# heng-hw/SpaCap3D

Hardware: AMD Instinct MI355X
Metric: scenes/sec (40k pts, 256 proposals) fwd+bwd (higher is better)
Workload: dtype f32; 1 GPU; cfg2: synthetic ScanRefer-shaped scans, 40000 pts x (xyz+1 ch), 256 proposals, 8 scenes/GPU; full training step (SpaCapNet fwd + loss + bwd + grad all-reduce + Adam); global_batch=8, parallelism=dp1, hip_graph=True, fps_prefetch_side_stream=True, prefetch_as_graph=True, reserved_cus_forward=8, geometry_prefetch=True, deferred_weight_gradients=True, params=9290918, allreduce_bytes=35572416

## Files before the change

include/spacap_hip.h:

```cpp
#ifndef SPACAP_HIP_H
#define SPACAP_HIP_H

#include <stddef.h>
#include <stdint.h>

#ifdef __cplusplus
extern "C" {
#endif

#define SPACAP_ABI_VERSION 5

#define SPACAP_OK 0
#define SPACAP_E_INVALID (-1)
#define SPACAP_E_LAUNCH (-2)
#define SPACAP_E_NO_DEVICE (-3)

typedef void *spacap_stream_t;

int spacap_abi_version(void);
const char *spacap_last_error(void);
int spacap_device_count(void);

int spacap_opt_n_threads(int work_size);

// ... 361 lines not shown
  float eps;
  uint64_t seed;
  const uint64_t *seed_dev;
  const float *res;
  float *x_out;
  const float *ln_a;
  const float *ln_b;
  float *n_out;
  float *stats;
  const float *x_ln;
  const float *g;
  float *part;
  const float *w2;
  const float *bias2;
  float *out2;
  int n2;
  int nparts;
  const float *attn_out;
  float *delta_out;
  int lq;
} spacap_tf_rows_args;
int spacap_tf_rows_f32(const spacap_tf_rows_args *args, spacap_stream_t stream);
int spacap_tf_rows_parts(long R);
int spacap_tf_ffn1_f32(const float *x, const float *W, const float *bias, long R, int N, float drop_p, uint64_t seed,
                       const uint64_t *seed_dev, float *h, spacap_stream_t stream);
int spacap_tf_ffn_f32(int mode, const float *x, const float *Wa, const float *Wb, const float *bias, const float *y, long R, int dff,
                      float drop_p, uint64_t seed, const uint64_t *seed_dev, float *hid, float *part, spacap_stream_t stream);
long spacap_tf_ffn_pieces_elems(int dff);
int spacap_tf_ffn_split_f32(const float *const *w1, const float *const *w2, void *const *pieces, int nlayers, int dff,
                            spacap_stream_t stream);
int spacap_tf_ffn_bf3_f32(int mode, const float *x, const void *pieces, const float *bias, const float *y, long R, int dff, float drop_p,
                          uint64_t seed, const uint64_t *seed_dev, float *hid, float *part, spacap_stream_t stream);
int spacap_decode_attn_f32(const float *qkv, float *kcache, float *vcache, long R, int h, int d_k, int T, int t, float scale,
                           float *out, spacap_stream_t stream);
size_t spacap_decode_word_workspace_bytes(long R, int V);
int spacap_decode_word_f32(const float *x, const void *Wp, const float *bias, long R, int V, const float *lut, float scale,
                           const float *pe_row, int64_t *ys, int ys_ld, int t_out, float *x_next, void *workspace,
                           spacap_stream_t stream);
int spacap_tf_gemm_splits(long R, int K, int N);
int spacap_tf_gemm_f32(const float *a, const float *W, long R, int K, int N, int trans_w, int nsplit, float *out,
                       spacap_stream_t stream);
int spacap_tf_dgrad_mask_f32(const float *g, const float *W, const float *y, float scale, long R, int K, int N, float *out,
                             spacap_stream_t stream);

int spacap_conv1x1_cm_supported(int CI, int CO, long N);
int spacap_conv1x1_cm_f32(int mode, const float *W, const float *in, const float *bias, int B, int CI, int CO, long N,
// ... 66 lines not shown
```

spacap3d_amd/_native.py:

```python
import ctypes
import os

import torch

_HERE = os.path.dirname(os.path.abspath(__file__))
LIB_PATH = os.path.join(_HERE, "lib", "libspacap_hip.so")
ABI_VERSION = 5

_i = ctypes.c_int
_l = ctypes.c_long
_f = ctypes.c_float
_p = ctypes.c_void_p
_u64 = ctypes.c_uint64

SIGNATURES = {
    "spacap_abi_version": (_i, []),
    "spacap_last_error": (ctypes.c_char_p, []),
    "spacap_device_count": (_i, []),
    "spacap_opt_n_threads": (_i, [_i]),
    "spacap_fps_workspace_bytes": (ctypes.c_size_t, [_i, _i]),
    "spacap_fps_f32": (_i, [_p, _i, _i, _i, _p, _p, _p]),
    "spacap_gather_points_f32": (_i, [_p, _p, _i, _i, _i, _i, _p, _p]),
    "spacap_gather_points_grad_f32": (_i, [_p, _p, _i, _i, _i, _i, _p, _p]),
    "spacap_ball_query_f32": (_i, [_p, _p, _i, _i, _i, _f, _i, _p, _p]),
# ... 141 lines not shown
    "spacap_rel_tail_bwd_nparts": (_i, [_l]),
    "spacap_rel_tail_bwd_f32": (_i, [_p, _p, _p, _l, _p, _p, _p]),
    "spacap_conv1x1_wgrad_slabs": (_i, [_i, _i, _i, _i]),
    "spacap_conv1x1_wgrad_f32": (_i, [_p, _p, _i, _i, _i, _i, _p, _p]),
    "spacap_conv1x1_wgrad_slabs_batched": (_i, [_i, _i, _i, _i]),
    "spacap_conv1x1_wgrad_batched_f32": (_i, [_p, _p, _p, _p, _p, _p, _p, _p, _p, _i, _p]),
    "spacap_linear_rows_supported": (_i, [_l, _i, _i]),
    "spacap_linear_rows_f32": (_i, [_p, _p, _p, _l, _i, _i, _i, _p, _p]),
    "spacap_linear_wgrad_slabs": (_i, [_l, _i, _i]),
    "spacap_linear_wgrad_f32": (_i, [_p, _p, _l, _i, _i, _i, _p, _p]),
    "spacap_linear_wgrad_nslab_f32": (_i, [_p, _p, _l, _i, _i, _i, _i, _p, _p]),
    "spacap_linear_wgrad_slabs_batched": (_i, [_l, _i, _i]),
    "spacap_linear_wgrad_batched_f32": (_i, [_p, _p, _p, _p, _p, _p, _p, _p, _i, _p]),
    "spacap_layernorm_fwd_f32": (_i, [_p, _p, _p, _l, _i, _f, _p, _p, _p]),
    "spacap_layernorm_bwd_workspace_bytes": (ctypes.c_size_t, [_l, _i]),
    "spacap_layernorm_bwd_f32": (_i, [_p, _p, _p, _p, _l, _i, _f, _p, _p, _p, _p, _p]),
    "spacap_layernorm_bwd_add_f32": (_i, [_p, _p, _p, _p, _p, _l, _i, _f, _p, _p, _p, _p, _p]),
    "spacap_proposal_decode_fwd_f32": (_i, [_p, _p, _p, _p, _i, _i, _i, _i, _i, _p, _p, _p, _p, _p, _p, _p, _p, _p]),
    "spacap_proposal_decode_bwd_f32": (_i, [_p, _p, _p, _p, _p, _i, _i, _i, _i, _i, _p, _p]),
    "spacap_loss_tail_fwd_f32": (_i, [_p, _p, _p, _p, _p, _p, _i, _p, _p, _p]),
    "spacap_loss_tail_bwd_f32": (_i, [_p, _p, _p, _p, _p]),
    "spacap_tf_rows_f32": (_i, [_p, _p]),
    "spacap_tf_rows_parts": (_i, [_l]),
    "spacap_tf_ffn1_f32": (_i, [_p, _p, _p, _l, _i, _f, _u64, _p, _p, _p]),
    "spacap_tf_ffn_f32": (_i, [_i, _p, _p, _p, _p, _p, _l, _i, _f, _u64, _p, _p, _p, _p]),
    "spacap_tf_ffn_pieces_elems": (_l, [_i]),
    "spacap_tf_ffn_split_f32": (_i, [_p, _p, _p, _i, _i, _p]),
    "spacap_tf_ffn_bf3_f32": (_i, [_i, _p, _p, _p, _p, _l, _i, _f, _u64, _p, _p, _p, _p]),
    "spacap_decode_attn_f32": (_i, [_p, _p, _p, _l, _i, _i, _i, _i, _f, _p, _p]),
    "spacap_decode_word_workspace_bytes": (ctypes.c_size_t, [_l, _i]),
    "spacap_decode_word_f32": (_i, [_p, _p, _p, _l, _i, _p, _f, _p, _p, _i, _i, _p, _p, _p]),
    "spacap_tf_gemm_splits": (_i, [_l, _i, _i]),
    "spacap_tf_gemm_f32": (_i, [_p, _p, _l, _i, _i, _i, _i, _p, _p]),
    "spacap_tf_dgrad_mask_f32": (_i, [_p, _p, _p, _f, _l, _i, _i, _p, _p]),
    "spacap_mha_fwd_f32": (_i, [_p, _p, _p] + [_l] * 9 + [_p, _l, _l, _p, _l, _l, _l]
                           + [_i] * 5 + [_f, _f, _u64, _p, _p, _p, _p, _p]),
    "spacap_mha_bwd_workspace_bytes": (ctypes.c_size_t, [_i, _i, _i]),
    "spacap_mha_bwd_delta_f32": (_i, [_p, _p, _p] + [_l] * 9 + [_p, _l, _l, _p, _l, _l, _l]
                                 + [_i] * 5 + [_f, _f, _u64, _p, _p, _p, _p, _p, _p, _p, _l, _p]),
    "spacap_mha_bwd_f32": (_i, [_p, _p, _p] + [_l] * 9 + [_p, _l, _l, _p, _l, _l, _l]
                           + [_i] * 5 + [_f, _f, _u64, _p, _p, _p, _p, _p, _p, _p, _p, _l, _p]),
}


class TfRowsArgs(ctypes.Structure):
    _fields_ = [("mode", _i), ("R", _l), ("a1", _p), ("w1", _p), ("bias1", _p), ("k1", _i), ("drop_p", _f), ("eps", _f),
                ("seed", _u64), ("seed_dev", _p), ("res", _p), ("x_out", _p), ("ln_a", _p), ("ln_b", _p), ("n_out", _p),
                ("stats", _p), ("x_ln", _p), ("g", _p), ("part", _p), ("w2", _p), ("bias2", _p), ("out2", _p), ("n2", _i), ("nparts", _i), ("attn_out", _p), ("delta_out", _p), ("lq", _i)]


def _load():
    if not os.path.exists(LIB_PATH):
        raise ImportError(
            f"{LIB_PATH} not found: the HIP extension is not built. Run "
            "`python -c 'import __graft_entry__ as g; g.build()'` (or `make -C spacap3d_amd/csrc`). "
            "spacap3d_amd has no CPU or PyTorch fallback for its native operators.")
    lib = ctypes.CDLL(LIB_PATH)
    for name, (res, args) in SIGNATURES.items():
        fn = getattr(lib, name)
        fn.restype = res
        fn.argtypes = args
    got = lib.spacap_abi_version()
    if got != ABI_VERSION:
        raise ImportError(f"libspacap_hip.so ABI {got} != expected {ABI_VERSION}: rebuild the extension")
    return lib


lib = _load()


def check(rc: int, what: str) -> None:
# ... 196 lines not shown
```

spacap3d_amd/tf_layer.py:

```python
import ctypes

import torch
from torch.autograd import Function

from ._native import TfRowsArgs, check, grad_slot, lib, linear_wgrad_partials, sum_slabs

D_MODEL = 128
ENABLED = True


def supported(d_model, d_ff):
    return d_model == D_MODEL and d_ff >= 128 and d_ff % 128 == 0


def _p(t):
    return t.data_ptr() if t is not None else None


def _rows(mode, R, dev, **kw):
    a = TfRowsArgs()
    a.mode, a.R = mode, R
    a.k1 = int(kw.pop("k1", 0))
    a.n2 = int(kw.pop("n2", 0))
    a.nparts = int(kw.pop("nparts", 0))
    a.lq = int(kw.pop("lq", 0))
    a.drop_p = float(kw.pop("drop_p", 0.0))
    a.eps = float(kw.pop("eps", 1e-6))
    a.seed = int(kw.pop("seed", 0))
    a.seed_dev = None
    if a.drop_p > 0.0:
        from .attention import rng_state
# ... 231 lines not shown
            if g_hpre is not None and g_parts is not None:
                gh, gp = g_hpre.reshape(R, dff).contiguous(), g_parts.contiguous()
                _rows(1, R, dev, a1=gp, nparts=gp.shape[0], **kw)
                dW1, db1 = _linear_grads(gh, n2, W1)
            elif g_hpre is not None:
                gh = g_hpre.reshape(R, dff).contiguous()
                parts, S = _split_product(gh, W1, False)
                _rows(1, R, dev, a1=parts, nparts=S, **kw)
                dW1, db1 = _linear_grads(gh, n2, W1)
            else:
                _rows(1, R, dev, g=torch.zeros(R, D_MODEL, dtype=torch.float32, device=dev), **kw)
            dln_a, dln_b = _ln_param_grads(part)
            dWo, dbo = _linear_grads(dy1, a.reshape(R, D_MODEL), Wo)
            dqkv = torch.empty_like(qc)
            base, gb = qc.data_ptr(), dqkv.data_ptr()
            check(lib.spacap_mha_bwd_delta_f32(base, base + hd * es, base + 2 * hd * es, *strides, *strides, *strides, _p(mask_u8),
                                               mask_sb, mask_sq, None, 0, 0, 0, B, heads, L, L, dk, scale, p_att, seed_att,
                                               rng_state(dev).data_ptr() if p_att > 0.0 else None, lse.data_ptr(), da.data_ptr(),
                                               delta.data_ptr(), gb, gb + hd * es, gb + 2 * hd * es, three, st),
                  "spacap_mha_bwd_delta_f32")
        return (dqkv, dx1, None, None, None, None, None, None, dWo, dbo, dln_a, dln_b, dW1, db1, None, None, None, None, None, None)


class Ffn2Ln(Function):

    @staticmethod
    def forward(ctx, h, parts, x1, W1, W2, b2, ln_a, ln_b, eps, p_sub, p_ffn, seed3, pw, pb, *routing):
        if not h.is_cuda:
            raise RuntimeError("CPU not supported")
        hc, xr, pc = h.contiguous(), x1.contiguous(), parts.contiguous()
        R, dev = xr.numel() // D_MODEL, xr.device
        last = pw is None
        with torch.cuda.device(dev):
            x2, n, stats = _new(dev, *xr.shape), _new(dev, *xr.shape), _new(dev, R, 2)
            kw = dict(a1=pc, nparts=pc.shape[0], bias1=b2, drop_p=p_sub, seed=seed3, res=xr, x_out=x2, ln_a=ln_a, ln_b=ln_b,
                      eps=eps, n_out=n, stats=stats)
            qkv = None
            if not last:
                qkv = _new(dev, *xr.shape[:-1], pw.shape[0])
                kw.update(w2=pw, bias2=pb, n2=pw.shape[0], out2=qkv)
            _rows(0, R, dev, **kw)
        ctx.save_for_backward(hc, x2, n, stats, ln_a, W1, W2, pw)
        ctx.meta = (float(eps), float(p_sub), float(p_ffn), int(seed3), last, [int(r.shape[0]) for r in routing[:3]])
        ctx.set_materialize_grads(False)
        return (n,) if last else (x2, qkv)

# ... 41 lines not shown


def stack_supported(layers, x):
    if not (ENABLED and x.is_cuda and x.dtype == torch.float32 and x.shape[-1] == D_MODEL and len(layers) > 0):
        return False
    for l in layers:
        ff, sa = l.feed_forward, l.self_attn
        if getattr(l, "early_guide", True) is not True or sa.h * sa.d_k != D_MODEL:
            return False
        if not supported(ff.w_1.in_features, ff.w_1.out_features) or ff.w_2.bias is None or ff.w_1.bias is None:
            return False
        if any(li.bias is None or not li.weight.is_contiguous() for li in sa.linears):
            return False
    return True


def decode_supported(layers, x, n_words):
    if not stack_supported(layers, x) or n_words + 1 > 32:
        return False
    dff = layers[0].feed_forward.w_1.out_features
    return all(l.self_attn.h == 8 and l.self_attn.d_k == 16 and l.feed_forward.w_1.out_features == dff for l in layers)


def run_stack(layers, final_norm, x, mask):
    from .attention import _next_seed, _prep_mask, self_attention_packed

    def drop(m):
        return float(m.p) if m.training else 0.0

    def seed(p):
        return _next_seed() if p > 0.0 else 0

    sub = lambda l: (l.sublayer[0], l.sublayer[-1])
    l0 = layers[0]
    if x.numel() // x.shape[-1] > FFN_BF3_MIN_ROWS:
        refresh_ffn_pieces(layers)
    pw, pb, routing = _packed(l0.self_attn)
    qkv, xres = LnQkv.apply(x, l0.sublayer[0].norm.a_2, l0.sublayer[0].norm.b_2, l0.sublayer[0].norm.eps, pw, pb, *routing)
    out = None
    for i, l in enumerate(layers):
        sa, ff = l.self_attn, l.feed_forward
        s_att, s_ffn = sub(l)
        need_p = sa.keep_value if sa.store_attn is None else (sa.store_attn or sa.keep_value)
        p1, pf, p3 = drop(s_att.dropout), drop(ff.dropout), drop(s_ffn.dropout)
        wo = sa.linears[-1]
        tail = (wo.weight, wo.bias, s_ffn.norm.a_2, s_ffn.norm.b_2, ff.w_1.weight, ff.w_1.bias, ff.w_2.weight, s_ffn.norm.eps, p1, pf)
        if not need_p and sa.d_k == 16 and sa.h == 8:
            B_, L_ = qkv.shape[0], qkv.shape[1]
            m8, msb, msq = _prep_mask(mask, B_, L_, L_)
            pa = float(sa.dropout.p) if sa.dropout.training else 0.0
            sa.attn = None
            x1, h, parts = AttnFfn1.apply(qkv, xres, m8, msb, msq, sa.h, pa, seed(pa), *tail, seed(p1), seed(pf))
        else:
            a, sa.attn = self_attention_packed(qkv, sa.h, mask=mask, dropout_p=sa.dropout.p, training=sa.dropout.training,
                                               need_p=need_p)
            if sa.keep_value:
                hd = sa.h * sa.d_k
                sa.value = qkv[..., 2 * hd:].view(qkv.shape[0], -1, sa.h, sa.d_k).transpose(1, 2)
            x1, h, parts = AttnOutFfn1.apply(a, xres, *tail, seed(p1), seed(pf))
# ... 80 lines not shown
```

Before: 1151 scenes/s.

## Fuse short-sequence transformer layer into single per-scene block kernels

Adds a new HIP kernel pair that, for sequences up to 32 tokens, runs the FFN-residual sum, LayerNorm, QKV projection, attention, output projection, residual and second LayerNorm in one workgroup per scene, with a matching fused backward. The Python stack routes through it when shapes are supported. The aim is to cut the many small kernel launches and global-memory round trips of the short transformer stack. In exchange it adds a large specialised kernel with one block per batch element, which on a batch of 8 leaves most CUs idle and may run slower than the multi-kernel path.

```diff
diff --git a/include/spacap_hip.h b/include/spacap_hip.h
--- a/include/spacap_hip.h
+++ b/include/spacap_hip.h
@@ -407,6 +407,56 @@
 } spacap_tf_rows_args;
 int spacap_tf_rows_f32(const spacap_tf_rows_args *args, spacap_stream_t stream);
 int spacap_tf_rows_parts(long R);
+typedef struct {
+  int B, L;
+  const uint64_t *seed_dev;
+  const float *parts;
+  int nparts;
+  const float *bias0;
+  float drop0;
+  uint64_t seed0;
+  const float *x;
+  float *x0;
+  const float *ln1_a;
+  const float *ln1_b;
+  float eps1;
+  float *n1;
+  float *stats1;
+  const float *wqkv;
+  const float *bqkv;
+  float *qkv;
+  const uint8_t *mask;
+  long mask_sb, mask_sq;
+  float att_scale;
+  float drop_att;
+  uint64_t seed_att;
+  float *attn;
+  float *lse;
+  const float *wo;
+  const float *bo;
+  float drop1;
+  uint64_t seed1;
+  const float *ln2_a;
+  const float *ln2_b;
+  float eps2;
+  float *x1;
+  float *n2;
+  float *stats2;
+  const float *gparts;
+  int ngparts;
+  const float *g_x1;
+  float *dy1;
+  float *part2;
+  float *dqkv;
+  float *dx;
+  float *part1;
+  float *dy0;
+} spacap_tf_short_args;
+int spacap_tf_short_supported(int L, int d_model, int h, int d_k);
+int spacap_tf_short_parts(int B);
+long spacap_tf_short_lds_bytes(int backward);
+int spacap_tf_short_fwd_f32(const spacap_tf_short_args *args, spacap_stream_t stream);
+int spacap_tf_short_bwd_f32(const spacap_tf_short_args *args, spacap_stream_t stream);
 int spacap_tf_ffn1_f32(const float *x, const float *W, const float *bias, long R, int N, float drop_p, uint64_t seed,
                        const uint64_t *seed_dev, float *h, spacap_stream_t stream);
 int spacap_tf_ffn_f32(int mode, const float *x, const float *Wa, const float *Wb, const float *bias, const float *y, long R, int dff,
diff --git a/spacap3d_amd/_native.py b/spacap3d_amd/_native.py
--- a/spacap3d_amd/_native.py
+++ b/spacap3d_amd/_native.py
@@ -187,6 +187,11 @@
     "spacap_loss_tail_bwd_f32": (_i, [_p, _p, _p, _p, _p]),
     "spacap_tf_rows_f32": (_i, [_p, _p]),
     "spacap_tf_rows_parts": (_i, [_l]),
+    "spacap_tf_short_supported": (_i, [_i, _i, _i, _i]),
+    "spacap_tf_short_parts": (_i, [_i]),
+    "spacap_tf_short_lds_bytes": (_l, [_i]),
+    "spacap_tf_short_fwd_f32": (_i, [_p, _p]),
+    "spacap_tf_short_bwd_f32": (_i, [_p, _p]),
     "spacap_tf_ffn1_f32": (_i, [_p, _p, _p, _l, _i, _f, _u64, _p, _p, _p]),
     "spacap_tf_ffn_f32": (_i, [_i, _p, _p, _p, _p, _p, _l, _i, _f, _u64, _p, _p, _p, _p]),
     "spacap_tf_ffn_pieces_elems": (_l, [_i]),
@@ -212,6 +217,15 @@
     _fields_ = [("mode", _i), ("R", _l), ("a1", _p), ("w1", _p), ("bias1", _p), ("k1", _i), ("drop_p", _f), ("eps", _f),
                 ("seed", _u64), ("seed_dev", _p), ("res", _p), ("x_out", _p), ("ln_a", _p), ("ln_b", _p), ("n_out", _p),
                 ("stats", _p), ("x_ln", _p), ("g", _p), ("part", _p), ("w2", _p), ("bias2", _p), ("out2", _p), ("n2", _i), ("nparts", _i), ("attn_out", _p), ("delta_out", _p), ("lq", _i)]
+
+
+class TfShortArgs(ctypes.Structure):
+    _fields_ = [("B", _i), ("L", _i), ("seed_dev", _p), ("parts", _p), ("nparts", _i), ("bias0", _p), ("drop0", _f), ("seed0", _u64),
+                ("x", _p), ("x0", _p), ("ln1_a", _p), ("ln1_b", _p), ("eps1", _f), ("n1", _p), ("stats1", _p), ("wqkv", _p),
+                ("bqkv", _p), ("qkv", _p), ("mask", _p), ("mask_sb", _l), ("mask_sq", _l), ("att_scale", _f), ("drop_att", _f),
+                ("seed_att", _u64), ("attn", _p), ("lse", _p), ("wo", _p), ("bo", _p), ("drop1", _f), ("seed1", _u64), ("ln2_a", _p),
+                ("ln2_b", _p), ("eps2", _f), ("x1", _p), ("n2", _p), ("stats2", _p), ("gparts", _p), ("ngparts", _i), ("g_x1", _p),
+                ("dy1", _p), ("part2", _p), ("dqkv", _p), ("dx", _p), ("part1", _p), ("dy0", _p)]
 
 
 def _load():
diff --git a/spacap3d_amd/csrc/tf_short.hip b/spacap3d_amd/csrc/tf_short.hip
--- /dev/null
+++ b/spacap3d_amd/csrc/tf_short.hip
@@ -0,0 +1,704 @@
+#include <math.h>
+
+#include "common.hpp"
+#include "mfma.hpp"
+
+namespace {
+
+using namespace spacap::mfma;
+using f32x2 = float __attribute__((ext_vector_type(2)));
+
+constexpr int D = 128;
+constexpr int NH = 8, DK = 16;
+constexpr int LMAX = 32;
+constexpr int LDT = D + 8;
+constexpr int QS = 3 * D + 4;
+constexpr int NTHR = 512;
+
+constexpr size_t FWD_LDS = sizeof(float) * (LMAX * LDT + LMAX * QS + 2 * 8 * 16);
+constexpr size_t BWD_LDS = sizeof(float) * (2 * LMAX * LDT + LMAX * QS + 2 * 8 * 16 + NH * LMAX);
+
+__device__ __forceinline__ f32x2 ld2(const float *p) { return *reinterpret_cast<const f32x2 *>(p); }
+
+struct DropSeed {
+  unsigned lo, hi;
+};
+__device__ __forceinline__ DropSeed make_seed(unsigned long long seed, const unsigned long long *seed_dev) {
+  const unsigned long long s = seed + (seed_dev ? *seed_dev * 0x9E3779B97F4A7C15ull : 0ull);
+  return DropSeed{(unsigned)s, (unsigned)(s >> 32)};
+}
+__device__ __forceinline__ unsigned hash32(unsigned long long idx, DropSeed s) {
+  unsigned h = (unsigned)idx ^ s.lo;
+  h += ((unsigned)(idx >> 32) ^ s.hi) * 0x9E3779B1u;
+  h ^= h >> 16;
+  h *= 0x85EBCA6Bu;
+  h ^= h >> 13;
+  h *= 0xC2B2AE35u;
+  h ^= h >> 16;
+  return h;
+}
+
+struct Drop {
+  unsigned thresh;
+  float scale;
+  unsigned long long seed;
+};
+
+struct ShortArgs {
+  int B, L;
+  const unsigned long long *seed_dev;
+  const float *parts;
+  int nparts;
+  const float *bias0;
+  Drop d0;
+  const float *x;
+  float *x0;
+  const float *ln1_a, *ln1_b;
+  float eps1;
+  float *n1, *stats1;
+  const float *wqkv, *bqkv;
+  float *qkv;
+  const uint8_t *mask;
+  long mask_sb, mask_sq;
+  float att_scale;
+  Drop da;
+  float *attn, *lse;
+  const float *wo, *bo;
+  Drop d1;
+  const float *ln2_a, *ln2_b;
+  float eps2;
+  float *x1, *n2, *stats2;
+  const float *gparts;
+  int ngparts;
+  const float *g_x1;
+  float *dy1, *part2, *dqkv, *dx, *part1, *dy0;
+};
+
+struct Place {
+  int lane, w, w4, mt, l15, lg, rl;
+  bool valid;
+  long row, rowc;
+};
+__device__ __forceinline__ Place place(int b, int L) {
+  Place p;
+  p.lane = threadIdx.x & 63, p.w = threadIdx.x >> 6, p.w4 = p.w & 3, p.mt = p.w >> 2, p.l15 = p.lane & 15, p.lg = p.lane >> 4;
+  p.rl = 16 * p.mt + p.l15;
+  p.valid = p.rl < L;
+  p.row = (long)b * L + p.rl;
+  p.rowc = p.valid ? p.row : (long)b * L + L - 1;
+  return p;
+}
+
+__device__ __forceinline__ float red4(const float *s_red, int k, int mt, int l15) {
+  const float *r = s_red + (k * 8 + 4 * mt) * 16 + l15;
+  return (r[0] + r[16]) + (r[32] + r[48]);
+}
+
+__device__ __forceinline__ f32x4 sum_parts(const float *pp, size_t ps, int nparts) {
+  f32x4 a = ld4(pp);
+  int sidx = 1;
+  for (; sidx + 7 < nparts; sidx += 8) {
+    f32x4 t[8];
+#pragma unroll
+    for (int u = 0; u < 8; ++u) t[u] = ld4(pp + (sidx + u) * ps);
+#pragma unroll
+    for (int u = 0; u < 8; ++u) a += t[u];
+  }
+  for (; sidx + 3 < nparts; sidx += 4) {
+    const f32x4 t0 = ld4(pp + sidx * ps), t1 = ld4(pp + (sidx + 1) * ps), t2 = ld4(pp + (sidx + 2) * ps), t3 = ld4(pp + (sidx + 3) * ps);
+    a += t0, a += t1, a += t2, a += t3;
+  }
+  for (; sidx < nparts; ++sidx) a += ld4(pp + sidx * ps);
+  return a;
+}
+
+__device__ __forceinline__ void ln_fwd(const Place &pl, const int *cb, const float (&xo)[2][4], const float *ln_a, const float *ln_b,
+                                       float eps, float *n_out, float *stats, float *s_red, float (&t_out)[2][4]) {
+  float s = 0.f;
+#pragma unroll
+  for (int g = 0; g < 2; ++g)
+#pragma unroll
+    for (int t = 0; t < 4; ++t) s += xo[g][t];
+  s += __shfl_xor(s, 16);
+  s += __shfl_xor(s, 32);
+  if (pl.lg == 0) s_red[(0 * 8 + pl.w) * 16 + pl.l15] = s;
+  __syncthreads();
+  const float mu = red4(s_red, 0, pl.mt, pl.l15) / (float)D;
+  float q = 0.f;
+#pragma unroll
+  for (int g = 0; g < 2; ++g)
+#pragma unroll
+    for (int t = 0; t < 4; ++t) {
+      const float c = xo[g][t] - mu;
+      q += c * c;
+    }
+  q += __shfl_xor(q, 16);
+  q += __shfl_xor(q, 32);
+  if (pl.lg == 0) s_red[(1 * 8 + pl.w) * 16 + pl.l15] = q;
+  __syncthreads();
+  const float var = red4(s_red, 1, pl.mt, pl.l15) / (float)(D - 1);
+  const float r = 1.0f / (sqrtf(var) + eps);
+#pragma unroll
+  for (int g = 0; g < 2; ++g) {
+    const f32x4 a4 = ld4(ln_a + cb[g]), b4 = ld4(ln_b + cb[g]);
+#pragma unroll
+    for (int t = 0; t < 4; ++t) t_out[g][t] = a4[t] * ((xo[g][t] - mu) * r) + b4[t];
+    if (pl.valid) st4(n_out + (size_t)pl.row * D + cb[g], f32x4{t_out[g][0], t_out[g][1], t_out[g][2], t_out[g][3]});
+  }
+  if (pl.valid && pl.w4 == 0 && pl.lg == 0) {
+    stats[pl.row * 2] = mu;
+    stats[pl.row * 2 + 1] = r;
+  }
+}
+
+__device__ __forceinline__ float logit(const ShortArgs &P, float dot, int b, int q, int key, bool &masked) {
+  const int L = P.L;
+  float s = dot * P.att_scale;
+  const int qc = q < L ? q : L - 1, kc = key < L ? key : L - 1;
+  masked = false;
+  if (P.mask && P.mask[b * P.mask_sb + qc * P.mask_sq + kc] == 0) {
+    s = -1e9f;
+    masked = true;
+  }
+  if (key >= L) s = -INFINITY;
+  return s;
+}
+__device__ __forceinline__ bool keep_att(const ShortArgs &P, DropSeed sd, int b, int hh, int q, int key) {
+  if (P.da.thresh == 0u) return true;
+  const unsigned long long idx = (((unsigned long long)b * NH + hh) * P.L + q) * (unsigned long long)P.L + key;
+  return hash32(idx, sd) >= P.da.thresh;
+}
+
+__global__ __launch_bounds__(NTHR) void tf_short_fwd_kernel(const ShortArgs P) {
+  extern __shared__ __attribute__((aligned(16))) unsigned char smem_raw[];
+  float *s_t = reinterpret_cast<float *>(smem_raw);
+  float *s_qkv = s_t + LMAX * LDT;
+  float *s_red = s_qkv + LMAX * QS;
+  const int b = blockIdx.x, L = P.L;
+  const Place pl = place(b, L);
+  const int l15 = pl.l15, lg = pl.lg, w4 = pl.w4;
+  const long R = (long)P.B * L;
+  int cb[2];
+#pragma unroll
+  for (int g = 0; g < 2; ++g) cb[g] = 32 * w4 + 16 * g + 4 * lg;
+
+  float xo[2][4], t_out[2][4];
+  {
+    const DropSeed sd = make_seed(P.d0.seed, P.seed_dev);
+#pragma unroll
+    for (int g = 0; g < 2; ++g) {
+      const f32x4 r4 = ld4(P.x + (size_t)pl.rowc * D + cb[g]);
+      if (P.parts != nullptr) {
+        const f32x4 v = sum_parts(P.parts + (size_t)pl.rowc * D + cb[g], (size_t)R * D, P.nparts);
+        f32x4 b4 = {0.f, 0.f, 0.f, 0.f};
+        if (P.bias0) b4 = ld4(P.bias0 + cb[g]);
+#pragma unroll
+        for (int t = 0; t < 4; ++t) {
+          float a = v[t] + b4[t];
+          if (P.d0.thresh != 0u) {
+            const bool keep = hash32((unsigned long long)pl.row * D + cb[g] + t, sd) >= P.d0.thresh;
+            a = keep ? a * P.d0.scale : 0.f;
+          }
+          xo[g][t] = r4[t] + a;
+        }
+        if (pl.valid) st4(P.x0 + (size_t)pl.row * D + cb[g], f32x4{xo[g][0], xo[g][1], xo[g][2], xo[g][3]});
+      } else {
+#pragma unroll
+        for (int t = 0; t < 4; ++t) xo[g][t] = r4[t];
+      }
+    }
+  }
+  ln_fwd(pl, cb, xo, P.ln1_a, P.ln1_b, P.eps1, P.n1, P.stats1, s_red, t_out);
+
+#pragma unroll
+  for (int g = 0; g < 2; ++g) st4(&s_t[pl.rl * LDT + cb[g]], f32x4{t_out[g][0], t_out[g][1], t_out[g][2], t_out[g][3]});
+  __syncthreads();
+  {
+    f32x4 at[8];
+#pragma unroll
+    for (int q = 0; q < 8; ++q) at[q] = ld4(&s_t[pl.rl * LDT + 16 * q + 4 * lg]);
+    const int n00 = 96 * w4;
+    const float *wp = P.wqkv + (size_t)(n00 + l15) * D + 4 * lg;
+#pragma unroll
+    for (int jt = 0; jt < 96; jt += 32) {
+      f32x4 x[8], y[8];
+#pragma unroll
+      for (int q = 0; q < 8; ++q) x[q] = ld4(wp + (size_t)jt * D + 16 * q), y[q] = ld4(wp + (size_t)(jt + 16) * D + 16 * q);
+      f32x4 acc0 = {0.f, 0.f, 0.f, 0.f}, acc1 = {0.f, 0.f, 0.f, 0.f};
+#pragma unroll
+      for (int q = 0; q < 8; ++q)
+#pragma unroll
+        for (int i = 0; i < 4; ++i) {
+          acc0 = MFMA16(x[q][i], at[q][i], acc0);
+          acc1 = MFMA16(y[q][i], at[q][i], acc1);
+        }
+      const int c0 = n00 + jt + 4 * lg;
+      if (P.bqkv) acc0 += ld4(P.bqkv + c0), acc1 += ld4(P.bqkv + c0 + 16);
+      if (pl.valid) {
+        st4(P.qkv + (size_t)pl.row * 3 * D + c0, acc0);
+        st4(P.qkv + (size_t)pl.row * 3 * D + c0 + 16, acc1);
+      }
+      st4(&s_qkv[pl.rl * QS + c0], acc0);
+      st4(&s_qkv[pl.rl * QS + c0 + 16], acc1);
+    }
+  }
+  __syncthreads();
+
+  {
+    const DropSeed sd = make_seed(P.da.seed, P.seed_dev);
+    const int lq = l15;
+#pragma unroll
+    for (int tk = 0; tk < 2; ++tk) {
+      const int id = 2 * pl.w + tk, hh = id >> 1, q0 = (id & 1) * 16;
+      if (q0 >= L) continue;
+      const int q = q0 + lq, qc = q < L ? q : L - 1;
+      const float *qp = s_qkv + qc * QS + hh * DK;
+      float qreg[DK / 4];
+#pragma unroll
+      for (int s = 0; s < DK / 4; ++s) qreg[s] = qp[4 * s + lg];
+      f32x4 acc[2];
+#pragma unroll
+      for (int t = 0; t < 2; ++t) {
+        acc[t] = f32x4{0.f, 0.f, 0.f, 0.f};
+        if (16 * t < L) {
+          const int key = 16 * t + lq;
+          const float *kp = s_qkv + (key < L ? key : L - 1) * QS + D + hh * DK;
+#pragma unroll
+          for (int s = 0; s < DK / 4; ++s) acc[t] = MFMA16(kp[4 * s + lg], qreg[s], acc[t]);
+        }
+      }
+      float m = -INFINITY;
+#pragma unroll
+      for (int t = 0; t < 2; ++t)
+#pragma unroll
+        for (int r = 0; r < 4; ++r) {
+          bool masked;
+          acc[t][r] = logit(P, acc[t][r], b, q, 16 * t + 4 * lg + r, masked);
+          m = fmaxf(m, acc[t][r]);
+        }
+      m = fmaxf(m, __shfl_xor(m, 16));
+      m = fmaxf(m, __shfl_xor(m, 32));
+      float l = 0.f;
+#pragma unroll
+      for (int t = 0; t < 2; ++t)
+#pragma unroll
+        for (int r = 0; r < 4; ++r) {
+          acc[t][r] = expf(acc[t][r] - m);
+          l += acc[t][r];
+        }
+      l += __shfl_xor(l, 16);
+      l += __shfl_xor(l, 32);
+      if (lg == 0 && q < L) {
+        float *st = P.lse + (((size_t)b * NH + hh) * L + q) * 2;
+        st[0] = m;
+        st[1] = l;
+      }
+#pragma unroll
+      for (int t = 0; t < 2; ++t)
+#pragma unroll
+        for (int r = 0; r < 4; ++r) {
+          float pv = acc[t][r] / l;
+          if (!keep_att(P, sd, b, hh, q, 16 * t + 4 * lg + r)) pv = 0.f; else pv *= P.da.scale;
+          acc[t][r] = pv;
+        }
+      f32x4 o = {0.f, 0.f, 0.f, 0.f};
+#pragma unroll
+      for (int t = 0; t < 2; ++t) {
+        if (16 * t < L) {
+#pragma unroll
+          for (int r = 0; r < 4; ++r) {
+            const int key = 16 * t + 4 * lg + r;
+            const float *vp = s_qkv + (key < L ? key : L - 1) * QS + 2 * D + hh * DK;
+            o = MFMA16(acc[t][r], vp[lq], o);
+          }
+        }
+      }
+#pragma unroll
+      for (int rr = 0; rr < 4; ++rr) {
+        const int qo = q0 + 4 * lg + rr;
+        s_t[qo * LDT + hh * DK + lq] = o[rr];
+        if (qo < L) P.attn[((size_t)b * L + qo) * D + hh * DK + lq] = o[rr];
+      }
+    }
+  }
+  __syncthreads();
+
+  {
+    f32x4 at[8], x[8], y[8];
+    const float *wp0 = P.wo + (size_t)(32 * w4 + l15) * D + 4 * lg, *wp1 = wp0 + (size_t)16 * D;
+#pragma unroll
+    for (int q = 0; q < 8; ++q) x[q] = ld4(wp0 + 16 * q), y[q] = ld4(wp1 + 16 * q), at[q] = ld4(&s_t[pl.rl * LDT + 16 * q + 4 * lg]);
+    f32x4 acc[2] = {f32x4{0.f, 0.f, 0.f, 0.f}, f32x4{0.f, 0.f, 0.f, 0.f}};
+#pragma unroll
+    for (int q = 0; q < 8; ++q)
+#pragma unroll
+      for (int i = 0; i < 4; ++i) {
+        acc[0] = MFMA16(x[q][i], at[q][i], acc[0]);
+        acc[1] = MFMA16(y[q][i], at[q][i], acc[1]);
+      }
+    const DropSeed sd = make_seed(P.d1.seed, P.seed_dev);
+#pragma unroll
+    for (int g = 0; g < 2; ++g) {
+      f32x4 b4 = {0.f, 0.f, 0.f, 0.f};
+      if (P.bo) b4 = ld4(P.bo + cb[g]);
+#pragma unroll
+      for (int t = 0; t < 4; ++t) {
+        float a = acc[g][t] + b4[t];
+        if (P.d1.thresh != 0u) {
+          const bool keep = hash32((unsigned long long)pl.row * D + cb[g] + t, sd) >= P.d1.thresh;
+          a = keep ? a * P.d1.scale : 0.f;
+        }
+        xo[g][t] = xo[g][t] + a;
+      }
+      if (pl.valid) st4(P.x1 + (size_t)pl.row * D + cb[g], f32x4{xo[g][0], xo[g][1], xo[g][2], xo[g][3]});
+    }
+  }
+  ln_fwd(pl, cb, xo, P.ln2_a, P.ln2_b, P.eps2, P.n2, P.stats2, s_red, t_out);
+}
+
+__device__ __forceinline__ void ln_bwd(const Place &pl, const int *cb, const float (&v)[2][4], const float *x_ln, const float *stats,
+                                       const float *ln_a, float eps, const float (&ad)[2][4], const Drop &dr, DropSeed sd, float *part,
+                                       float *s_red, float (&dx)[2][4], float (&dy)[2][4]) {
+  const float mu = stats[pl.rowc * 2], r = stats[pl.rowc * 2 + 1];
+  float dn[2][4], xc[2][4], dxh[2][4], s1 = 0.f, s2 = 0.f;
+#pragma unroll
+  for (int g = 0; g < 2; ++g) {
+    const f32x4 x4 = ld4(x_ln + (size_t)pl.rowc * D + cb[g]), a4 = ld4(ln_a + cb[g]);
+#pragma unroll
+    for (int t = 0; t < 4; ++t) {
+      dn[g][t] = pl.valid ? v[g][t] : 0.f;
+      xc[g][t] = x4[t] - mu;
+      dxh[g][t] = dn[g][t] * a4[t];
+      s1 += dxh[g][t];
+      s2 += dxh[g][t] * xc[g][t];
+    }
+  }
+  s1 += __shfl_xor(s1, 16);
+  s1 += __shfl_xor(s1, 32);
+  s2 += __shfl_xor(s2, 16);
+  s2 += __shfl_xor(s2, 32);
+  if (pl.lg == 0) s_red[(0 * 8 + pl.w) * 16 + pl.l15] = s1, s_red[(1 * 8 + pl.w) * 16 + pl.l15] = s2;
+  __syncthreads();
+  s1 = red4(s_red, 0, pl.mt, pl.l15);
+  s2 = red4(s_red, 1, pl.mt, pl.l15);
+  const float sdv = 1.0f / r - eps;
+  const float c2 = -(s2 * r * r) / (sdv * (float)(D - 1));
+  const float c1 = r * s1 / (float)D;
+#pragma unroll
+  for (int g = 0; g < 2; ++g) {
+#pragma unroll
+    for (int t = 0; t < 4; ++t) {
+      dx[g][t] = r * dxh[g][t] + c2 * xc[g][t] - c1 + ad[g][t];
+      float y = dx[g][t];
+      if (dr.thresh != 0u) {
+        const bool keep = hash32((unsigned long long)pl.row * D + cb[g] + t, sd) >= dr.thresh;
+        y = keep ? y * dr.scale : 0.f;
+      }
+      dy[g][t] = pl.valid ? y : 0.f;
+    }
+#pragma unroll
+    for (int t = 0; t < 4; ++t) {
+      float pa = dn[g][t] * (xc[g][t] * r), pb = dn[g][t];
+#pragma unroll
+      for (int o = 1; o < 16; o <<= 1) {
+        pa += __shfl_xor(pa, o);
+        pb += __shfl_xor(pb, o);
+      }
+      if (pl.l15 == 0) {
+        part[cb[g] + t] = pa;
+        part[D + cb[g] + t] = pb;
+      }
+    }
+  }
+}
+
+__global__ __launch_bounds__(NTHR) void tf_short_bwd_kernel(const ShortArgs P) {
+  extern __shared__ __attribute__((aligned(16))) unsigned char smem_raw[];
+  float *s_t = reinterpret_cast<float *>(smem_raw);
+  float *s_da = s_t + LMAX * LDT;
+  float *s_qkv = s_da + LMAX * LDT;
+  float *s_red = s_qkv + LMAX * QS;
+  float *s_delta = s_red + 2 * 8 * 16;
+  const int b = blockIdx.x, L = P.L;
+  const Place pl = place(b, L);
+  const int l15 = pl.l15, lg = pl.lg, w4 = pl.w4;
+  const long R = (long)P.B * L;
+  int cb[2];
+#pragma unroll
+  for (int g = 0; g < 2; ++g) cb[g] = 32 * w4 + 8 * lg + 4 * g;
+
+  for (int e = threadIdx.x; e < LMAX * (3 * D / 4); e += NTHR) {
+    const int r = e / (3 * D / 4), c = 4 * (e - r * (3 * D / 4));
+    st4(&s_qkv[r * QS + c], ld4(P.qkv + ((size_t)b * L + (r < L ? r : L - 1)) * 3 * D + c));
+  }
+
+  float v[2][4], ad[2][4], dx1[2][4], t_out[2][4];
+#pragma unroll
+  for (int g = 0; g < 2; ++g) {
+    const f32x4 a = sum_parts(P.gparts + (size_t)pl.rowc * D + cb[g], (size_t)R * D, P.ngparts);
+    f32x4 r4 = {0.f, 0.f, 0.f, 0.f};
+    if (P.g_x1) r4 = ld4(P.g_x1 + (size_t)pl.rowc * D + cb[g]);
+#pragma unroll
+    for (int t = 0; t < 4; ++t) v[g][t] = a[t], ad[g][t] = r4[t];
+  }
+  ln_bwd(pl, cb, v, P.x1, P.stats2, P.ln2_a, P.eps2, ad, P.d1, make_seed(P.d1.seed, P.seed_dev),
+         P.part2 + (size_t)(2 * b + pl.mt) * 2 * D, s_red, dx1, t_out);
+#pragma unroll
+  for (int g = 0; g < 2; ++g) {
+    const f32x4 y4 = {t_out[g][0], t_out[g][1], t_out[g][2], t_out[g][3]};
+    if (pl.valid) st4(P.dy1 + (size_t)pl.row * D + cb[g], y4);
+    st4(&s_t[pl.rl * LDT + cb[g]], y4);
+  }
+  __syncthreads();
+
+  {
+    f32x4 at[8];
+    f32x2 wv[32];
+    const float *wp = P.wo + (size_t)(4 * lg) * D + 32 * w4 + 2 * l15;
+#pragma unroll
+    for (int q = 0; q < 8; ++q) {
+      at[q] = ld4(&s_t[pl.rl * LDT + 16 * q + 4 * lg]);
+#pragma unroll
+      for (int i = 0; i < 4; ++i) wv[q * 4 + i] = ld2(wp + (size_t)(16 * q + i) * D);
+    }
+    f32x4 acc[2] = {f32x4{0.f, 0.f, 0.f, 0.f}, f32x4{0.f, 0.f, 0.f, 0.f}};
+#pragma unroll
+    for (int q = 0; q < 8; ++q)
+#pragma unroll
+      for (int i = 0; i < 4; ++i) {
+        acc[0] = MFMA16(wv[q * 4 + i][0], at[q][i], acc[0]);
+        acc[1] = MFMA16(wv[q * 4 + i][1], at[q][i], acc[1]);
+      }
+    float dsum = 0.f;
+#pragma unroll
+    for (int g = 0; g < 2; ++g) {
+      const f32x4 o = {acc[0][2 * g], acc[1][2 * g], acc[0][2 * g + 1], acc[1][2 * g + 1]};
+      st4(&s_da[pl.rl * LDT + cb[g]], o);
+      const f32x4 a4 = ld4(P.attn + (size_t)pl.rowc * D + cb[g]);
+      dsum += (o[0] * a4[0] + o[1] * a4[1]) + (o[2] * a4[2] + o[3] * a4[3]);
+    }
+    dsum += __shfl_xor(dsum, 16);
+    if ((lg & 1) == 0) s_delta[(2 * w4 + (lg >> 1)) * LMAX + pl.rl] = dsum;
+  }
+  __syncthreads();
+
+  f32x4 dq[2], dk[2], dv[2];
+  {
+    const DropSeed sd = make_seed(P.da.seed, P.seed_dev);
+    const int lq = l15;
+#pragma unroll
+    for (int tk = 0; tk < 2; ++tk) {
+      const int id = 2 * pl.w + tk, hh = id >> 1, t0 = (id & 1) * 16;
+      dq[tk] = dk[tk] = dv[tk] = f32x4{0.f, 0.f, 0.f, 0.f};
+      if (t0 >= L) continue;
+      const float *stb = P.lse + ((size_t)b * NH + hh) * L * 2;
+      const float *delb = s_delta + hh * LMAX;
+      {
+        const int q = t0 + lq, qc = q < L ? q : L - 1;
+        const float *qp = s_qkv + qc * QS + hh * DK, *dop = s_da + qc * LDT + hh * DK;
+        float qreg[DK / 4], doreg[DK / 4];
+#pragma unroll
+        for (int s = 0; s < DK / 4; ++s) qreg[s] = qp[4 * s + lg], doreg[s] = dop[4 * s + lg];
+        const float m = stb[qc * 2], inv_l = 1.0f / stb[qc * 2 + 1];
+        const float delta = delb[qc];
+        f32x4 p[2], dp[2];
+#pragma unroll
+        for (int t = 0; t < 2; ++t) {
+          p[t] = dp[t] = f32x4{0.f, 0.f, 0.f, 0.f};
+          if (16 * t < L) {
+            const int keyl = 16 * t + lq, kcl = keyl < L ? keyl : L - 1;
+            const float *kp = s_qkv + kcl * QS + D + hh * DK, *vp = s_qkv + kcl * QS + 2 * D + hh * DK;
+#pragma unroll
+            for (int s = 0; s < DK / 4; ++s) {
+              p[t] = MFMA16(kp[4 * s + lg], qreg[s], p[t]);
+              dp[t] = MFMA16(vp[4 * s + lg], doreg[s], dp[t]);
+            }
+#pragma unroll
+            for (int r = 0; r < 4; ++r) {
+              const int key = 16 * t + 4 * lg + r;
+              bool masked;
+              const float s = logit(P, p[t][r], b, q, key, masked);
+              const float pr = (key < L) ? expf(s - m) * inv_l : 0.f;
+              float g = dp[t][r];
+              g = keep_att(P, sd, b, hh, q, key) ? g * P.da.scale : 0.f;
+              p[t][r] = pr;
+              dp[t][r] = (masked || key >= L) ? NAN : g;
+            }
+          }
+        }
+#pragma unroll
+        for (int t = 0; t < 2; ++t) {
+          if (16 * t < L) {
+#pragma unroll
+            for (int r = 0; r < 4; ++r) {
+              const int key = 16 * t + 4 * lg + r;
+              const float g = dp[t][r];
+              const float ds = (g != g) ? 0.f : p[t][r] * (g - delta) * P.att_scale;
+              const float *kp = s_qkv + (key < L ? key : L - 1) * QS + D + hh * DK;
+              dq[tk] = MFMA16(ds, kp[lq], dq[tk]);
+            }
+          }
+        }
+      }
+      {
+        const int key = t0 + lq, kc = key < L ? key : L - 1;
+        const float *kp = s_qkv + kc * QS + D + hh * DK, *vp = s_qkv + kc * QS + 2 * D + hh * DK;
+        float kreg[DK / 4], vreg[DK / 4];
+#pragma unroll
+        for (int s = 0; s < DK / 4; ++s) kreg[s] = kp[4 * s + lg], vreg[s] = vp[4 * s + lg];
+        for (int qt = 0; qt * 16 < L; ++qt) {
+          const int qa = qt * 16 + lq, qac = qa < L ? qa : L - 1;
+          const float *qp = s_qkv + qac * QS + hh * DK, *dop = s_da + qac * LDT + hh * DK;
+          f32x4 s4 = {0.f, 0.f, 0.f, 0.f}, g4 = {0.f, 0.f, 0.f, 0.f};
+#pragma unroll
+          for (int s = 0; s < DK / 4; ++s) {
+            s4 = MFMA16(qp[4 * s + lg], kreg[s], s4);
+            g4 = MFMA16(dop[4 * s + lg], vreg[s], g4);
+          }
+#pragma unroll
+          for (int r = 0; r < 4; ++r) {
+            const int q = qt * 16 + 4 * lg + r, qc = q < L ? q : L - 1;
+            const bool valid = (q < L) && (key < L);
+            bool masked;
+            const float s = logit(P, s4[r], b, q, key, masked);
+            const float pr = valid ? expf(s - stb[qc * 2]) / stb[qc * 2 + 1] : 0.f;
+            float g = g4[r];
+            const bool keep = keep_att(P, sd, b, hh, q, key);
+            g = keep ? g * P.da.scale : 0.f;
+            const float pd = keep ? pr * P.da.scale : 0.f;
+            const float ds = (masked || !valid) ? 0.f : pr * (g - delb[qc]) * P.att_scale;
+            const float *qr = s_qkv + qc * QS + hh * DK, *dor = s_da + qc * LDT + hh * DK;
+            dk[tk] = MFMA16(ds, qr[lq], dk[tk]);
+            dv[tk] = MFMA16(valid ? pd : 0.f, dor[lq], dv[tk]);
+          }
+        }
+      }
+    }
+  }
+  __syncthreads();
+#pragma unroll
+  for (int tk = 0; tk < 2; ++tk) {
+    const int id = 2 * pl.w + tk, hh = id >> 1, t0 = (id & 1) * 16;
+    if (t0 >= L) continue;
+#pragma unroll
+    for (int rr = 0; rr < 4; ++rr) {
+      const int ro = t0 + 4 * lg + rr;
+      float *sp = s_qkv + ro * QS + hh * DK + l15;
+      sp[0] = dq[tk][rr], sp[D] = dk[tk][rr], sp[2 * D] = dv[tk][rr];
+      if (ro < L) {
+        float *op = P.dqkv + ((size_t)b * L + ro) * 3 * D + hh * DK + l15;
+        op[0] = dq[tk][rr], op[D] = dk[tk][rr], op[2 * D] = dv[tk][rr];
+      }
+    }
+  }
+  __syncthreads();
+
+  {
+    f32x4 acc[2] = {f32x4{0.f, 0.f, 0.f, 0.f}, f32x4{0.f, 0.f, 0.f, 0.f}};
+    const float *ap = s_qkv + pl.rl * QS + 4 * lg;
+    const float *wp = P.wqkv + (size_t)(4 * lg) * D + 32 * w4 + 2 * l15;
+#pragma unroll 1
+    for (int kc = 0; kc < 3 * D; kc += 128) {
+      f32x4 a[8];
+      f32x2 x[32];
+#pragma unroll
+      for (int q = 0; q < 8; ++q) {
+        a[q] = ld4(ap + kc + 16 * q);
+#pragma unroll
+        for (int i = 0; i < 4; ++i) x[q * 4 + i] = ld2(wp + (size_t)(kc + 16 * q + i) * D);
+      }
+#pragma unroll
+      for (int q = 0; q < 8; ++q)
+#pragma unroll
+        for (int i = 0; i < 4; ++i) {
+          acc[0] = MFMA16(x[q * 4 + i][0], a[q][i], acc[0]);
+          acc[1] = MFMA16(x[q * 4 + i][1], a[q][i], acc[1]);
+        }
+    }
+#pragma unroll
+    for (int i = 0; i < 2; ++i)
+#pragma unroll
+      for (int u = 0; u < 4; ++u) v[u >> 1][2 * (u & 1) + i] = acc[i][u];
+  }
+  float dx0[2][4];
+  ln_bwd(pl, cb, v, P.x0, P.stats1, P.ln1_a, P.eps1, dx1, P.d0, make_seed(P.d0.seed, P.seed_dev),
+         P.part1 + (size_t)(2 * b + pl.mt) * 2 * D, s_red, dx0, t_out);
+  if (pl.valid) {
+#pragma unroll
+    for (int g = 0; g < 2; ++g) {
+      st4(P.dx + (size_t)pl.row * D + cb[g], f32x4{dx0[g][0], dx0[g][1], dx0[g][2], dx0[g][3]});
+      if (P.dy0) st4(P.dy0 + (size_t)pl.row * D + cb[g], f32x4{t_out[g][0], t_out[g][1], t_out[g][2], t_out[g][3]});
+    }
+  }
+}
+
+inline bool drop_params(float p, uint64_t seed, Drop &d) {
+  if (!(p >= 0.f && p < 1.f)) return false;
+  d.thresh = p > 0.f ? (unsigned)((double)p * 4294967296.0) : 0u;
+  d.scale = 1.0f / (1.0f - p);
+  d.seed = seed;
+  return true;
+}
+inline bool al16(const void *p) { return (reinterpret_cast<uintptr_t>(p) & 15) == 0; }
+
+int fill(ShortArgs &P, const spacap_tf_short_args *a, const char *what) {
+  SPACAP_REQUIRE(a != nullptr, "%s: null argument block", what);
+  SPACAP_REQUIRE(a->B >= 0 && a->B <= 65535 && a->L >= 1 && a->L <= LMAX, "%s: (B=%d, L=%d) unsupported (L <= %d)", what, a->B, a->L, LMAX);
+  P.B = a->B, P.L = a->L;
+  P.seed_dev = reinterpret_cast<const unsigned long long *>(a->seed_dev);
+  SPACAP_REQUIRE(drop_params(a->drop0, a->seed0, P.d0) && drop_params(a->drop_att, a->seed_att, P.da) &&
+                     drop_params(a->drop1, a->seed1, P.d1), "%s: bad dropout probability", what);
+  P.parts = a->parts, P.nparts = a->nparts, P.bias0 = a->bias0, P.x = a->x, P.x0 = a->x0;
+  P.ln1_a = a->ln1_a, P.ln1_b = a->ln1_b, P.eps1 = a->eps1, P.n1 = a->n1, P.stats1 = a->stats1;
+  P.wqkv = a->wqkv, P.bqkv = a->bqkv, P.qkv = a->qkv;
+  P.mask = a->mask, P.mask_sb = a->mask_sb, P.mask_sq = a->mask_sq, P.att_scale = a->att_scale;
+  P.attn = a->attn, P.lse = a->lse, P.wo = a->wo, P.bo = a->bo;
+  P.ln2_a = a->ln2_a, P.ln2_b = a->ln2_b, P.eps2 = a->eps2, P.x1 = a->x1, P.n2 = a->n2, P.stats2 = a->stats2;
+  P.gparts = a->gparts, P.ngparts = a->ngparts, P.g_x1 = a->g_x1;
+  P.dy1 = a->dy1, P.part2 = a->part2, P.dqkv = a->dqkv, P.dx = a->dx, P.part1 = a->part1, P.dy0 = a->dy0;
+  SPACAP_REQUIRE(P.nparts >= 0 && (P.parts != nullptr) == (P.nparts > 0), "%s: parts and nparts = %d disagree", what, P.nparts);
+  SPACAP_REQUIRE(P.ln1_a && P.wqkv && P.qkv && P.attn && P.lse && P.wo && P.ln2_a && P.x1 && P.stats1 && P.stats2,
+                 "%s: null pointer", what);
+  SPACAP_REQUIRE(al16(P.parts) && al16(P.bias0) && al16(P.x) && al16(P.x0) && al16(P.ln1_a) && al16(P.ln1_b) && al16(P.n1) &&
+                     al16(P.wqkv) && al16(P.bqkv) && al16(P.qkv) && al16(P.attn) && al16(P.wo) && al16(P.bo) && al16(P.ln2_a) &&
+                     al16(P.ln2_b) && al16(P.x1) && al16(P.n2) && al16(P.gparts) && al16(P.g_x1) && al16(P.dy1) && al16(P.dqkv) &&
+                     al16(P.dx) && al16(P.dy0),
+                 "%s: pointers must be 16-byte aligned", what);
+  return SPACAP_OK;
+}
+
+}
+
+extern "C" int spacap_tf_short_supported(int L, int d_model, int h, int d_k) {
+  return L >= 1 && L <= LMAX && d_model == D && h == NH && d_k == DK;
+}
+extern "C" int spacap_tf_short_parts(int B) { return 2 * (B > 0 ? B : 0); }
+extern "C" long spacap_tf_short_lds_bytes(int backward) { return (long)(backward ? BWD_LDS : FWD_LDS); }
+
+extern "C" int spacap_tf_short_fwd_f32(const spacap_tf_short_args *a, spacap_stream_t stream) {
+  const char *what = "spacap_tf_short_fwd_f32";
+  ShortArgs P;
+  const int rc = fill(P, a, what);
+  if (rc) return rc;
+  if (P.B == 0) return SPACAP_OK;
+  SPACAP_REQUIRE(P.x && P.ln1_b && P.ln2_b && P.n1 && P.n2 && (!P.parts || P.x0), "%s: null pointer", what);
+  static unsigned long long lds_ok = 0;
+  SPACAP_CHECK_HIP(spacap::allow_dynamic_lds(reinterpret_cast<const void *>(&tf_short_fwd_kernel), (int)FWD_LDS, lds_ok), what);
+  hipLaunchKernelGGL(tf_short_fwd_kernel, dim3((unsigned)P.B), dim3(NTHR), FWD_LDS, spacap::as_stream(stream), P);
+  SPACAP_CHECK_LAUNCH(what);
+  return SPACAP_OK;
+}
+
+extern "C" int spacap_tf_short_bwd_f32(const spacap_tf_short_args *a, spacap_stream_t stream) {
+  const char *what = "spacap_tf_short_bwd_f32";
+  ShortArgs P;
+  const int rc = fill(P, a, what);
+  if (rc) return rc;
+  if (P.B == 0) return SPACAP_OK;
+  SPACAP_REQUIRE(P.x0 && P.gparts && P.ngparts > 0 && P.dy1 && P.part2 && P.dqkv && P.dx && P.part1, "%s: null pointer", what);
+  static unsigned long long lds_ok = 0;
+  SPACAP_CHECK_HIP(spacap::allow_dynamic_lds(reinterpret_cast<const void *>(&tf_short_bwd_kernel), (int)BWD_LDS, lds_ok), what);
+  hipLaunchKernelGGL(tf_short_bwd_kernel, dim3((unsigned)P.B), dim3(NTHR), BWD_LDS, spacap::as_stream(stream), P);
+  SPACAP_CHECK_LAUNCH(what);
+  return SPACAP_OK;
+}
diff --git a/spacap3d_amd/tf_layer.py b/spacap3d_amd/tf_layer.py
--- a/spacap3d_amd/tf_layer.py
+++ b/spacap3d_amd/tf_layer.py
@@ -3,10 +3,11 @@
 import torch
 from torch.autograd import Function
 
-from ._native import TfRowsArgs, check, grad_slot, lib, linear_wgrad_partials, sum_slabs
+from ._native import TfRowsArgs, TfShortArgs, check, grad_slot, lib, linear_wgrad_partials, sum_slabs
 
 D_MODEL = 128
 ENABLED = True
+SHORT = True
 
 
 def supported(d_model, d_ff):
@@ -284,6 +285,101 @@
         return (dqkv, dx1, None, None, None, None, None, None, dWo, dbo, dln_a, dln_b, dW1, db1, None, None, None, None, None, None)
 
 
+class ShortAttnFfn1(Function):
+
+    @staticmethod
+    def forward(ctx, xres, hprev, parts_prev, W1p, W2p, b2p, p3, pfp, seed3, ln1_a, ln1_b, eps1, pw, pb, mask_u8, mask_sb, mask_sq,
+                heads, p_att, seed_att, Wo, bo, ln2_a, ln2_b, W1, b1, W2, eps2, p_sub, p_ffn, seed1, seed2, *routing):
+        if not xres.is_cuda:
+            raise RuntimeError("CPU not supported")
+        import math
+        from .attention import rng_state
+        xr = xres.contiguous()
+        B, L, _ = xr.shape
+        R, dev = B * L, xr.device
+        dff = W1.shape[0]
+        first = parts_prev is None
+        a = TfShortArgs()
+        a.B, a.L = B, L
+        a.seed_dev = rng_state(dev).data_ptr() if max(p3, p_att, p_sub) > 0.0 else None
+        with torch.cuda.device(dev):
+            x0 = xr if first else _new(dev, B, L, D_MODEL)
+            n1, st1, qkv = _new(dev, R, D_MODEL), _new(dev, R, 2), _new(dev, B, L, 3 * D_MODEL)
+            att, lse = _new(dev, R, D_MODEL), _new(dev, B, heads, L, 2)
+            x1, n2, st2 = _new(dev, B, L, D_MODEL), _new(dev, R, D_MODEL), _new(dev, R, 2)
+            if not first:
+                pc = parts_prev.contiguous()
+                a.parts, a.nparts, a.bias0, a.drop0, a.seed0, a.x0 = pc.data_ptr(), pc.shape[0], _p(b2p), float(p3), int(seed3), x0.data_ptr()
+            a.x, a.ln1_a, a.ln1_b, a.eps1, a.n1, a.stats1 = xr.data_ptr(), _p(ln1_a), _p(ln1_b), float(eps1), n1.data_ptr(), st1.data_ptr()
+            a.wqkv, a.bqkv, a.qkv = pw.data_ptr(), _p(pb), qkv.data_ptr()
+            a.mask, a.mask_sb, a.mask_sq = _p(mask_u8), mask_sb, mask_sq
+            a.att_scale, a.drop_att, a.seed_att = 1.0 / math.sqrt(D_MODEL // heads), float(p_att), int(seed_att)
+            a.attn, a.lse, a.wo, a.bo, a.drop1, a.seed1 = att.data_ptr(), lse.data_ptr(), Wo.data_ptr(), _p(bo), float(p_sub), int(seed1)
+            a.ln2_a, a.ln2_b, a.eps2, a.x1, a.n2, a.stats2 = _p(ln2_a), _p(ln2_b), float(eps2), x1.data_ptr(), n2.data_ptr(), st2.data_ptr()
+            check(lib.spacap_tf_short_fwd_f32(ctypes.byref(a), torch.cuda.current_stream(dev).cuda_stream), "spacap_tf_short_fwd_f32")
+            h, parts = _ffn(0, n2, W1, W2, b1, None, dff, p_ffn, seed2, dev)
+        ctx.save_for_backward(x0, n1, st1, qkv, att, lse, x1, n2, st2, mask_u8, hprev, ln1_a, pw, Wo, ln2_a, W1, W1p, W2p)
+        ctx.meta = (float(eps1), float(eps2), float(p3), float(pfp or 0.0), int(seed3), float(p_att), int(seed_att), float(p_sub),
+                    int(seed1), int(heads), mask_sb, mask_sq, first, [int(r.shape[0]) for r in routing[:3]])
+        ctx.set_materialize_grads(False)
+        return x1, h.view(B, L, dff), parts
+
+    @staticmethod
+    def backward(ctx, g_x1, g_hpre, g_parts):
+        import math
+        from .attention import rng_state
+        x0, n1, st1, qkv, att, lse, x1, n2, st2, mask_u8, hprev, ln1_a, pw, Wo, ln2_a, W1, W1p, W2p = ctx.saved_tensors
+        eps1, eps2, p3, pfp, seed3, p_att, seed_att, p_sub, seed1, heads, mask_sb, mask_sq, first, rows = ctx.meta
+        B, L, _ = x1.shape
+        R, dev = B * L, x1.device
+        dff = W1.shape[0]
+        a = TfShortArgs()
+        a.B, a.L = B, L
+        a.seed_dev = rng_state(dev).data_ptr() if max(p3, p_att, p_sub) > 0.0 else None
+        with torch.cuda.device(dev):
+            dW1 = db1 = None
+            if g_hpre is not None and g_parts is not None:
+                gh, gp = g_hpre.reshape(R, dff).contiguous(), g_parts.contiguous()
+                dW1, db1 = _linear_grads(gh, n2, W1)
+            elif g_hpre is not None:
+                gh = g_hpre.reshape(R, dff).contiguous()
+                gp, _ = _split_product(gh, W1, False)
+                dW1, db1 = _linear_grads(gh, n2, W1)
+            else:
+                gp = torch.zeros(1, R, D_MODEL, dtype=torch.float32, device=dev)
+            gx = g_x1.contiguous() if g_x1 is not None else None
+            nsl = int(lib.spacap_tf_short_parts(B))
+            dy1, dqkv, dx = _new(dev, R, D_MODEL), _new(dev, R, 3 * D_MODEL), _new(dev, B, L, D_MODEL)
+            part1, part2 = _new(dev, nsl, 2 * D_MODEL), _new(dev, nsl, 2 * D_MODEL)
+            dy0 = None if first else _new(dev, R, D_MODEL)
+            a.x0, a.stats1, a.ln1_a, a.eps1, a.wqkv, a.qkv = x0.data_ptr(), st1.data_ptr(), ln1_a.data_ptr(), eps1, pw.data_ptr(), qkv.data_ptr()
+            a.mask, a.mask_sb, a.mask_sq = _p(mask_u8), mask_sb, mask_sq
+            a.att_scale, a.drop_att, a.seed_att = 1.0 / math.sqrt(D_MODEL // heads), p_att, seed_att
+            a.attn, a.lse, a.wo, a.drop1, a.seed1 = att.data_ptr(), lse.data_ptr(), Wo.data_ptr(), p_sub, seed1
+            a.ln2_a, a.eps2, a.x1, a.stats2 = ln2_a.data_ptr(), eps2, x1.data_ptr(), st2.data_ptr()
+            a.drop0, a.seed0 = (0.0, 0) if first else (p3, seed3)
+            a.gparts, a.ngparts, a.g_x1 = gp.data_ptr(), gp.shape[0], _p(gx)
+            a.dy1, a.part2, a.dqkv, a.dx, a.part1, a.dy0 = dy1.data_ptr(), part2.data_ptr(), dqkv.data_ptr(), dx.data_ptr(), \
+                part1.data_ptr(), _p(dy0)
+            check(lib.spacap_tf_short_bwd_f32(ctypes.byref(a), torch.cuda.current_stream(dev).cuda_stream), "spacap_tf_short_bwd_f32")
+            dln2_a, dln2_b = _ln_param_grads(part2)
+            dln1_a, dln1_b = _ln_param_grads(part1)
+            dWo, dbo = _linear_grads(dy1, att, Wo)
+            dw, dbias = _linear_grads(dqkv, n1, pw)
+            dh = gparts = dW2p = db2p = None
+            if not first:
+                dffp = W2p.shape[1]
+                hflat = hprev.reshape(R, dffp)
+                dh, gparts = _ffn(1, dy0, W2p, W1p, None, hflat, dffp, pfp, 0, dev)
+                dW2p, db2p = _linear_grads(dy0, hflat, W2p)
+                dh = dh.view_as(hprev)
+        head = (dx, dh, gparts, None, dW2p, db2p, None, None, None, dln1_a, dln1_b, None)
+        tail = (None, None, None, None, None, None, dWo, dbo, dln2_a, dln2_b, dW1, db1, None, None, None, None, None, None)
+        if rows:
+            return head + (None, None) + tail + _route_qkv(dw, dbias, rows)
+        return head + (dw, dbias) + tail
+
+
 class Ffn2Ln(Function):
 
     @staticmethod
@@ -371,6 +467,40 @@
     return all(l.self_attn.h == 8 and l.self_attn.d_k == 16 and l.feed_forward.w_1.out_features == dff for l in layers)
 
 
+def short_supported(layers, x):
+    if not SHORT or x.dim() != 3:
+        return False
+    for l in layers:
+        sa = l.self_attn
+        if sa.keep_value or sa.store_attn or not lib.spacap_tf_short_supported(x.shape[1], x.shape[2], sa.h, sa.d_k):
+            return False
+    return x.shape[0] > 0
+
+
+def _run_short_stack(layers, final_norm, x, mask, drop, seed):
+    from .attention import _prep_mask
+    B, L = x.shape[0], x.shape[1]
+    m8, msb, msq = _prep_mask(mask, B, L, L)
+    xres, h, parts, prev = x, None, None, (None, None, None, 0.0, 0.0, 0)
+    for l in layers:
+        sa, ff = l.self_attn, l.feed_forward
+        s_att, s_ffn = l.sublayer[0], l.sublayer[-1]
+        p1, pf, p3 = drop(s_att.dropout), drop(ff.dropout), drop(s_ffn.dropout)
+        pa = float(sa.dropout.p) if sa.dropout.training else 0.0
+        pw, pb, routing = _packed(sa)
+        wo = sa.linears[-1]
+        sa.attn = None
+        seed_att, seed1, seed2 = seed(pa), seed(p1), seed(pf)
+        xres, h, parts = ShortAttnFfn1.apply(xres, h, parts, *prev, s_att.norm.a_2, s_att.norm.b_2, s_att.norm.eps, pw, pb, m8, msb, msq,
+                                             sa.h, pa, seed_att, wo.weight, wo.bias, s_ffn.norm.a_2, s_ffn.norm.b_2, ff.w_1.weight,
+                                             ff.w_1.bias, ff.w_2.weight, s_ffn.norm.eps, p1, pf, seed1, seed2, *routing)
+        prev = (ff.w_1.weight, ff.w_2.weight, ff.w_2.bias, p3, pf, seed(p3))
+    ff = layers[-1].feed_forward
+    (out,) = Ffn2Ln.apply(h, parts, xres, ff.w_1.weight, ff.w_2.weight, ff.w_2.bias, final_norm.a_2, final_norm.b_2, final_norm.eps,
+                          prev[3], prev[4], prev[5], None, None)
+    return out
+
+
 def run_stack(layers, final_norm, x, mask):
     from .attention import _next_seed, _prep_mask, self_attention_packed
 
@@ -384,6 +514,8 @@
     l0 = layers[0]
     if x.numel() // x.shape[-1] > FFN_BF3_MIN_ROWS:
         refresh_ffn_pieces(layers)
+    if short_supported(layers, x):
+        return _run_short_stack(layers, final_norm, x, mask, drop, seed)
     pw, pb, routing = _packed(l0.self_attn)
     qkv, xres = LnQkv.apply(x, l0.sublayer[0].norm.a_2, l0.sublayer[0].norm.b_2, l0.sublayer[0].norm.eps, pw, pb, *routing)
     out = None
```

New measurement: 1131 scenes/s. -1.7%, worse.
